# mimbres/neural-audio-fp

Hardware: NVIDIA B200
Metric: search_queries_per_s (higher is better)
Workload: dtype bf16 scan, f32 re-rank

## Files before the change

neural-audio-fp_b200/csrc/flat_search.cu:

```cuda
#include <cfloat>
#include <climits>
#include <cstdlib>
#include <cstring>
#include <algorithm>
#include <vector>

#include "index.h"
#include "ptx.cuh"

namespace nafp {

__global__ void flat_convert_rows_kernel(const float* __restrict__ x32, __nv_bfloat16* __restrict__ x16,
                                         float* __restrict__ hn, int32_t* __restrict__ maxn2, int64_t row0,
                                         int64_t n) {
    const int lane = threadIdx.x & 31;
    const int64_t warp = (static_cast<int64_t>(blockIdx.x) * blockDim.x + threadIdx.x) >> 5;
    const int64_t nwarps = (static_cast<int64_t>(gridDim.x) * blockDim.x) >> 5;
    float mx = 0.f;
    for (int64_t r = row0 + warp; r < row0 + n; r += nwarps) {
        const float4 v = reinterpret_cast<const float4*>(x32 + r * D128)[lane];
        __nv_bfloat162 a = __floats2bfloat162_rn(v.x, v.y);
        __nv_bfloat162 b = __floats2bfloat162_rn(v.z, v.w);
        uint2 packed;
        packed.x = *reinterpret_cast<uint32_t*>(&a);
// ... 1 lines not shown
        reinterpret_cast<uint2*>(x16 + r * D128)[lane] = packed;
        float ss = v.x * v.x + v.y * v.y + v.z * v.z + v.w * v.w;
#pragma unroll
        for (int o = 16; o > 0; o >>= 1) ss += __shfl_xor_sync(0xffffffffu, ss, o);
        if (lane == 0) hn[r] = 0.5f * ss;
        mx = fmaxf(mx, ss);
    }
    if (lane == 0 && mx > 0.f) atomicMax(maxn2, __float_as_int(mx));
}

__global__ void flat_fill_kernel(float* hn, int64_t from, int64_t to, float v) {
    int64_t i = from + static_cast<int64_t>(blockIdx.x) * blockDim.x + threadIdx.x;
    if (i < to) hn[i] = v;
}

__global__ void flat_prep_kernel(const float* __restrict__ q_all, const int32_t* __restrict__ src_list, int src_off,
                                 int64_t p0, int nq, int nq_pad, int grid_scan,
                                 __nv_bfloat16* __restrict__ qbf, float* __restrict__ q32,
                                 float* __restrict__ qn2, int32_t* __restrict__ Mx, int32_t* __restrict__ Tg,
                                 int32_t* __restrict__ flags, int64_t* __restrict__ gidx, int32_t* __restrict__ tile_counter) {
    const int lane = threadIdx.x & 31;
    const int row = (blockIdx.x * blockDim.x + threadIdx.x) >> 5;
    if (blockIdx.x == 0 && threadIdx.x == 0) *tile_counter = 0;
    if (row >= nq_pad) return;
    int64_t g = -1;
    if (row < nq) g = src_list ? static_cast<int64_t>(src_list[src_off + row]) : p0 + row;
    float4 v = make_float4(0.f, 0.f, 0.f, 0.f);
    if (g >= 0) v = reinterpret_cast<const float4*>(q_all + g * D128)[lane];
    __nv_bfloat162 a = __floats2bfloat162_rn(v.x, v.y);
    __nv_bfloat162 b = __floats2bfloat162_rn(v.z, v.w);
    uint2 packed;
    packed.x = *reinterpret_cast<uint32_t*>(&a);
    packed.y = *reinterpret_cast<uint32_t*>(&b);
    reinterpret_cast<uint2*>(qbf + row * D128)[lane] = packed;
    reinterpret_cast<float4*>(q32 + row * D128)[lane] = v;
    float ss = v.x * v.x + v.y * v.y + v.z * v.z + v.w * v.w;
#pragma unroll
    for (int o = 16; o > 0; o >>= 1) ss += __shfl_xor_sync(0xffffffffu, ss, o);
    if (lane == 0) {
        qn2[row] = ss;
        Tg[row] = INT_MIN;
        flags[row] = 0;
        gidx[row] = g;
    }
    for (int c = lane; c < grid_scan; c += 32) Mx[row * grid_scan + c] = INT_MIN;
}

constexpr int RING_SLOTS = 4;
constexpr int EPI_WARPS = 16;
constexpr int SCAN_THREADS = (3 + EPI_WARPS) * 32;
constexpr int TMA_WARP = EPI_WARPS + 1, MMA_WARP = EPI_WARPS + 2;
constexpr int EPI_PARTS = EPI_WARPS / 4;
constexpr int PART_COLS = SCAN_TILE / EPI_PARTS;
constexpr int SLOT_BYTES = SCAN_TILE * 128;
constexpr int BOX_BYTES = TILE_ROWS * 128;
constexpr int Q_KB_BYTES = NQ_CTA * 128;
constexpr int Q_BYTES_MAX = 2 * Q_KB_BYTES;
constexpr int H_RING = 4;
constexpr int WARM_TILES = 8;
constexpr int SCAN_SMEM = Q_BYTES_MAX + RING_SLOTS * SLOT_BYTES + H_RING * SCAN_TILE * 4 + 3 * NQ_CTA * 4 + 256 + 1024;
constexpr uint16_t PAIR_MASK = 0b11, RANK0_MASK = 0b01;
constexpr int NEG_INF_ORD = static_cast<int>(0x807FFFFFu);
static_assert(PART_COLS == 64, "epilogue reads two 32-column chunks per unit");

struct ScanBars {
    uint64_t full[RING_SLOTS];
    uint64_t empty[RING_SLOTS];
    uint64_t tfull[2];
    uint64_t tempty[2];
    uint64_t qfull;
    uint32_t tmem_base;
    int done;
    int tile_of[8];
};

__device__ __forceinline__ void smem_red_max(int* p, int v) {
    asm volatile("red.shared.max.s32 [%0], %1;" ::"r"(smem_u32(p)), "r"(v) : "memory");
}
__device__ __forceinline__ int smem_atom_inc(int* p) {
    int old;
    asm volatile("atom.shared.add.u32 %0, [%1], 1;" : "=r"(old) : "r"(smem_u32(p)) : "memory");
    return old;
}
__device__ __forceinline__ int smem_atom_add(int* p, int v) {
    int old;
    asm volatile("atom.shared.add.u32 %0, [%1], %2;" : "=r"(old) : "r"(smem_u32(p)), "r"(v) : "memory");
    return old;
}
__device__ __forceinline__ int smem_ld_volatile(const int* p) {
    int v;
    asm volatile("ld.volatile.shared.s32 %0, [%1];" : "=r"(v) : "r"(smem_u32(p)) : "memory");
    return v;
}
__device__ __forceinline__ float fmax3(float a, float b, float c) {
    float d;
    asm("max.f32 %0, %1, %2, %3;" : "=f"(d) : "f"(a), "f"(b), "f"(c));
    return d;
}
__device__ __forceinline__ void mbar_arrive_lane0(uint64_t* bar, int lane) {
    asm volatile(
        "{\n\t.reg .pred p;\n\tsetp.eq.s32 p, %1, 0;\n\t@p mbarrier.arrive.shared::cta.b64 _, [%0];\n\t}" ::"r"(smem_u32(bar)),
        "r"(lane)
        : "memory");
}
template <bool EDGE>
__device__ __forceinline__ void scan_chunk_hits(const uint32_t (&v)[32], const float* __restrict__ hc, float t_exact, int nvalid,
                                                uint32_t rbase, int* cnt_q, int* lmax_q, uint64_t* pool_q) {
    uint32_t m = 0;
    float best = -INFINITY;
#pragma unroll
    for (int j = 0; j < 32; ++j) {
        if (!EDGE || j < nvalid) {
            const float sj = __uint_as_float(v[j]) - hc[j];
            m |= (sj > t_exact) ? (1u << j) : 0u;
            best = fmaxf(best, sj);
        }
    }
    if (m) {
        smem_red_max(lmax_q, f2ord(best));
        int pos = smem_atom_add(cnt_q, __popc(m));
        while (m) {
            const int j = __ffs(m) - 1;
            m &= m - 1;
            if (pos < POOL_CAP) pool_q[pos] = rbase + j;
            ++pos;
        }
    }
}

__global__ void __launch_bounds__(SCAN_THREADS, 1)
flat_scan_kernel(const __grid_constant__ CUtensorMap tmap_q, const __grid_constant__ CUtensorMap tmap_db,
                 const float* __restrict__ hn, int32_t* __restrict__ tile_counter, int64_t n_search, int n_tiles, int nq,
                 int n_half, int kg, int32_t* __restrict__ Mx, int32_t* __restrict__ Tg, uint64_t* __restrict__ pool,
                 int32_t* __restrict__ cnt, int32_t* __restrict__ flags, int32_t* __restrict__ dbg_first, int tune) {
    extern __shared__ uint8_t smem_raw[];
    uint8_t* smem = reinterpret_cast<uint8_t*>((reinterpret_cast<uintptr_t>(smem_raw) + 1023) & ~uintptr_t(1023));
    uint8_t* q_s = smem;
    uint8_t* b_s = smem + Q_BYTES_MAX;
    float* h_s = reinterpret_cast<float*>(b_s + RING_SLOTS * SLOT_BYTES);
    int* lmax_s = reinterpret_cast<int*>(h_s + H_RING * SCAN_TILE);
    int* cnt_s = lmax_s + 2 * NQ_CTA;
    ScanBars* bars = reinterpret_cast<ScanBars*>(cnt_s + NQ_CTA);

    const int warp = threadIdx.x >> 5;
    const int lane = threadIdx.x & 31;
    const int G = gridDim.x;
    const int cta = blockIdx.x;
    const int rank = cta & 1, clu = cta >> 1, C = G >> 1;
    const int qrow0 = rank * n_half * 128;
    const int warm_cap = ((tune >> 8) & 15) ? ((tune >> 8) & 15) : WARM_TILES;
    const int warm = (tune & 2) ? 1 : max(1, min(warm_cap, n_tiles / C));

    for (int i = threadIdx.x; i < NQ_CTA; i += blockDim.x) {
        lmax_s[i] = INT_MIN;
        lmax_s[NQ_CTA + i] = INT_MIN;
        cnt_s[i] = 0;
    }
    if (threadIdx.x == 0) {
        tma_prefetch_desc(&tmap_q);
        tma_prefetch_desc(&tmap_db);
        for (int s = 0; s < RING_SLOTS; ++s) {
            mbar_init(&bars->full[s], 1);
            mbar_init(&bars->empty[s], 2);
        }
        for (int a = 0; a < 2; ++a) {
            mbar_init(&bars->tfull[a], 1);
            mbar_init(&bars->tempty[a], EPI_WARPS);
        }
        mbar_init(&bars->qfull, 1);
        bars->done = 0;
        mbar_fence_init();
    }
    if (warp == MMA_WARP) {
        tmem_alloc(&bars->tmem_base, 512);
        tmem_relinquish();
    }
    tc_fence_before();
    cluster_sync();
    tc_fence_after();
    const uint32_t tmem_base = __shfl_sync(0xffffffffu, bars->tmem_base, 0);

    if (warp == TMA_WARP) {
        if (lane == 0) {
            const int q_rows = n_half * 128;
            mbar_arrive_expect_tx(&bars->qfull, 2u * q_rows * 128u);
            for (int kb = 0; kb < 2; ++kb)
                for (int r0 = 0; r0 < q_rows; r0 += 32)
                    tma_load_2d(q_s + kb * Q_KB_BYTES + r0 * 128, &tmap_q, &bars->qfull, kb * 64, qrow0 + r0);
        }
        if (lane == 0 && rank == 0) {
            const uint32_t peer_full0 = map_shared_rank(&bars->full[0], 1);
            const uint32_t peer_tile_of0 = map_shared_rank(&bars->tile_of[0], 1);
            int tile = clu;
            int revisit = -1;
            int nxt = warm * C + atomicAdd(tile_counter, 1);
            int i = 0;
            for (;; ++i) {
                const int kc0 = 2 * i;
                const uint32_t ph = (kc0 / RING_SLOTS) & 1;
                const int s0 = kc0 % RING_SLOTS;
                mbar_wait_parked(&bars->empty[s0], ph ^ 1);
                bars->tile_of[i & 7] = tile;
                mbar_arrive_expect_tx_remote(peer_full0 + 8 * s0, (tile < 0 ? 0 : SLOT_BYTES + SCAN_TILE * 4) + 4);
                st_async_remote(peer_tile_of0 + 4 * (i & 7), tile, peer_full0 + 8 * s0);
                if (tile < 0) {
                    mbar_arrive(&bars->full[s0]);
                    break;
                }
#pragma unroll
                for (int kb = 0; kb < 2; ++kb) {
                    const int s = s0 + kb;
                    if (kb == 1) {
                        mbar_wait_parked(&bars->empty[s], ph ^ 1);
                        mbar_arrive_expect_tx_remote(peer_full0 + 8 * s, SLOT_BYTES);
                    }
                    mbar_arrive_expect_tx(&bars->full[s], SLOT_BYTES + (kb == 0 ? SCAN_TILE * 4 : 0));
                    if (kb == 0)
                        bulk_load_1d_multicast(h_s + (i % H_RING) * SCAN_TILE, hn + static_cast<int64_t>(tile) * SCAN_TILE,
                                               SCAN_TILE * 4, &bars->full[s], PAIR_MASK);
                    uint8_t* dst = b_s + s * SLOT_BYTES;
                    tma_load_2d_multicast(dst, &tmap_db, &bars->full[s], kb * 64, tile * SCAN_TILE, PAIR_MASK);
                    tma_load_2d_multicast(dst + BOX_BYTES, &tmap_db, &bars->full[s], kb * 64, tile * SCAN_TILE + TILE_ROWS,
                                          PAIR_MASK);
                }
                if (i + 1 < warm) {
                    tile = clu + (i + 1) * C;
                } else if (revisit < 0 && nxt < n_tiles) {
                    tile = nxt;
                    nxt = warm * C + atomicAdd(tile_counter, 1);
                } else {
                    ++revisit;
                    tile = revisit < warm ? clu + revisit * C : -1;
                }
            }
            for (int kc = 2 * i + 1; kc < 2 * i + RING_SLOTS; ++kc)
                mbar_wait_parked(&bars->empty[kc % RING_SLOTS], ((kc / RING_SLOTS) & 1) ^ 1);
        }
        __syncwarp();
    } else if (warp == MMA_WARP) {
        const bool leader = elect_one();
        const uint32_t idesc = umma_idesc_f16(1u, 128u, static_cast<uint32_t>(SCAN_TILE));
        const uint64_t adesc0 = umma_desc_sw128(smem_u32(q_s));
        const uint64_t bdesc0 = umma_desc_sw128(smem_u32(b_s));
        mbar_wait_parked(&bars->qfull, 0);
        uint32_t uc = 0;
        bool more = true;
        for (int i = 0; more; ++i) {
            const int s0 = (2 * i) % RING_SLOTS, s1 = s0 + 1;
            const uint32_t ph = ((2 * i) / RING_SLOTS) & 1;
            for (int hq = 0; hq < n_half; ++hq, ++uc) {
                const int acc = uc & 1;
                const uint32_t aph = (uc >> 1) & 1;
                const bool last = hq == n_half - 1;
                mbar_wait_parked(&bars->tempty[acc], aph ^ 1);
                if (hq == 0) {
                    mbar_wait_parked_cluster(&bars->full[s0], ph);
                    if (smem_ld_volatile(&bars->tile_of[i & 7]) < 0) {
                        if (leader) tc_commit(&bars->tfull[acc]);
                        __syncwarp();
                        more = false;
                        break;
                    }
                }
                tc_fence_after();
                const uint32_t d_tmem = tmem_base + acc * SCAN_TILE;
                const uint64_t a_kb0 = adesc0 + static_cast<uint64_t>((hq * (128 * 128)) >> 4);
                const uint64_t a_kb1 = a_kb0 + static_cast<uint64_t>(Q_KB_BYTES >> 4);
                const uint64_t b_kb0 = bdesc0 + static_cast<uint64_t>((s0 * SLOT_BYTES) >> 4);
                const uint64_t b_kb1 = b_kb0 + static_cast<uint64_t>(SLOT_BYTES >> 4);
                if (leader) {
#pragma unroll
                    for (int j = 0; j < 4; ++j) tc_mma_f16(d_tmem, a_kb0 + 2 * j, b_kb0 + 2 * j, idesc, j != 0 ? 1u : 0u);
                    if (last) tc_commit_multicast(&bars->empty[s0], RANK0_MASK);
                }
                if (hq == 0) {
                    mbar_wait_parked_cluster(&bars->full[s1], ph);
                    tc_fence_after();
                }
                if (leader) {
#pragma unroll
                    for (int j = 0; j < 4; ++j) tc_mma_f16(d_tmem, a_kb1 + 2 * j, b_kb1 + 2 * j, idesc, 1u);
                    if (last) tc_commit_multicast(&bars->empty[s1], RANK0_MASK);
                    tc_commit(&bars->tfull[acc]);
                }
                __syncwarp();
            }
        }
        __syncwarp();
    } else if (warp < EPI_WARPS) {
        const int qd = warp & 3;
        const int e = warp;
        const int part = e >> 2;
        constexpr int QPW = NQ_CTA / EPI_WARPS;
        static_assert(2 * QPW == 32, "one lane per (query, column half) when maxima are published");
        const int q_rows = n_half * 128;
        int* lmax_part = lmax_s + (part >> 1) * NQ_CTA;
        const float NEG_INF = -INFINITY;
        int pub = INT_MIN;
        int thr_ord[2] = {NEG_INF_ORD, NEG_INF_ORD};
        float t_exact[2], t_pre[2];
        bool active[2];
#pragma unroll
        for (int hq = 0; hq < 2; ++hq) {
            active[hq] = hq < n_half && qrow0 + (hq * 128 + qd * 32 + lane) < nq;
            t_exact[hq] = active[hq] ? NEG_INF : INFINITY;
            t_pre[hq] = t_exact[hq];
        }
        uint64_t* my_pool = pool + static_cast<int64_t>(cta) * NQ_CTA * POOL_CAP;
        const uint32_t ns32 = static_cast<uint32_t>(n_search);
        auto load_thresholds = [&](int (&tg)[2]) {
#pragma unroll
            for (int hq = 0; hq < 2; ++hq) tg[hq] = active[hq] ? ld_relaxed(&Tg[qrow0 + hq * 128 + qd * 32 + lane]) : INT_MIN;
        };
        auto apply_thresholds = [&](const int (&tg)[2], int i) -> bool {
            bool valid = true;
#pragma unroll
            for (int hq = 0; hq < 2; ++hq) {
                if (active[hq]) {
                    if (tg[hq] > thr_ord[hq]) {
                        if (dbg_first && part == 0 && thr_ord[hq] == NEG_INF_ORD)
                            dbg_first[cta * NQ_MAX + qrow0 + hq * 128 + qd * 32 + lane] = i;
                        thr_ord[hq] = tg[hq];
                        const float t = ord2f(tg[hq]);
                        t_exact[hq] = t;
                        t_pre[hq] = t - fabsf(t) * (1.f / 1048576.f) - 1e-37f;
                    }
                    valid = valid && (thr_ord[hq] > NEG_INF_ORD);
                }
            }
            return __all_sync(0xffffffffu, valid);
        };
        auto publish_maxima = [&]() {
            const int ql = e * QPW + (lane % QPW), half = lane / QPW;
            if (ql < q_rows && qrow0 + ql < nq) {
                const int m = smem_ld_volatile(&lmax_s[half * NQ_CTA + ql]);
                if (m > pub) {
                    st_relaxed(&Mx[(qrow0 + ql) * G + 2 * clu + half], m);
                    pub = m;
                }
            }
        };
        const bool probe = dbg_first != nullptr && threadIdx.x == 0 && nq <= NQ_MAX - 8;
        unsigned long long t_start = 0;
        if (probe) asm volatile("mov.u64 %0, %%globaltimer;" : "=l"(t_start));
        auto stamp = [&](int slot) {
            if (probe) {
                unsigned long long t;
                asm volatile("mov.u64 %0, %%globaltimer;" : "=l"(t));
                dbg_first[cta * NQ_MAX + NQ_MAX - 8 + slot] = static_cast<int>(t - t_start);
            }
        };
        const uint32_t tlane = tmem_base + (static_cast<uint32_t>(qd * 32) << 16) + part * PART_COLS;
        uint32_t uc = 0;

        for (int w = 0; w < warm; ++w) {
            const uint32_t row0 = static_cast<uint32_t>(clu + w * C) * SCAN_TILE + part * PART_COLS;
            const float* h_part = h_s + (w % H_RING) * SCAN_TILE + part * PART_COLS;
            bool edge = (static_cast<uint32_t>(clu + w * C) + 1u) * SCAN_TILE > ns32 || (tune & 4);
            float hx = 0.f;
            for (int hq = 0; hq < n_half; ++hq, ++uc) {
                const int acc = uc & 1;
                mbar_wait_parked(&bars->tfull[acc], (uc >> 1) & 1);
                if (hq == 0 && !edge) {
                    const float a = h_part[lane], b = h_part[32 + lane];
                    const float hmax_w = __uint_as_float(__reduce_max_sync(0xffffffffu, __float_as_uint(fmaxf(a, b))));
                    const float hmin_w = __uint_as_float(__reduce_min_sync(0xffffffffu, __float_as_uint(fminf(a, b))));
                    hx = hmax_w * (1.f + 1.f / 1048576.f);
                    edge = !(hmax_w - hmin_w <= hmax_w * (1.f / 262144.f));
                }
                tc_fence_after();
                float munit = NEG_INF;
#pragma unroll 1
                for (int c = 0; c < PART_COLS / 32; ++c) {
                    uint32_t v[32];
                    tmem_ld_32x32(tlane + acc * SCAN_TILE + c * 32, v);
                    tc_wait_ld();
                    if (!edge) {
                        float gm[4];
#pragma unroll
                        for (int g = 0; g < 4; ++g) {
                            float m = fmax3(__uint_as_float(v[8 * g]), __uint_as_float(v[8 * g + 1]), __uint_as_float(v[8 * g + 2]));
                            m = fmax3(m, __uint_as_float(v[8 * g + 3]), __uint_as_float(v[8 * g + 4]));
                            m = fmax3(m, __uint_as_float(v[8 * g + 5]), __uint_as_float(v[8 * g + 6]));
                            gm[g] = fmaxf(m, __uint_as_float(v[8 * g + 7]));
                        }
                        munit = fmaxf(munit, fmaxf(fmax3(gm[0], gm[1], gm[2]), gm[3]) - hx);
                    } else {
                        const float* hc = h_part + c * 32;
                        const int nvalid = static_cast<int>(min(ns32 - min(ns32, row0 + c * 32), 32u));
#pragma unroll
                        for (int j = 0; j < 32; ++j)
                            if (j < nvalid) munit = fmaxf(munit, __uint_as_float(v[j]) - hc[j]);
                    }
                }
                if (hq == 0 ? active[0] : active[1]) smem_red_max(&lmax_part[hq * 128 + qd * 32 + lane], f2ord(munit));
                tc_fence_before();
                __syncwarp();
                mbar_arrive_lane0(&bars->tempty[acc], lane);
            }
            publish_maxima();
            if (w == 0) stamp(0);
        }
        {
            int tg[2];
            bool ok = false;
            for (int spin = 0; spin < 4096 && !ok; ++spin) {
                publish_maxima();
                load_thresholds(tg);
                ok = apply_thresholds(tg, 1);
                if (!ok) __nanosleep(100);
            }
            stamp(1);
        }
        for (int i = warm;; ++i) {
            int tg[2] = {INT_MIN, INT_MIN};
            const bool rf = i > warm && (((tune & 8) && i < warm + 32) || (i & 3) == 0);
            if (rf) load_thresholds(tg);
            const float* h_part = h_s + (i % H_RING) * SCAN_TILE + part * PART_COLS;
            uint32_t row0 = 0;
            float hm = 0.f;
            bool end = false, edge = false;
            for (int hq = 0; hq < n_half; ++hq, ++uc) {
                const int acc = uc & 1;
                mbar_wait_parked(&bars->tfull[acc], (uc >> 1) & 1);
                if (hq == 0) {
                    const int tile = smem_ld_volatile(&bars->tile_of[i & 7]);
                    if (tile < 0) {
                        end = true;
                        break;
                    }
                    row0 = static_cast<uint32_t>(tile) * SCAN_TILE + part * PART_COLS;
                    const float hmin_w =
                        __uint_as_float(__reduce_min_sync(0xffffffffu, __float_as_uint(fminf(h_part[lane], h_part[32 + lane]))));
                    hm = hmin_w * (1.f - 1.f / 1048576.f);
                    edge = (static_cast<uint32_t>(tile) + 1u) * SCAN_TILE > ns32 || (tune & 4);
                }
                const float tp = (hq == 0 ? t_pre[0] : t_pre[1]) + hm;
                tc_fence_after();
                const uint32_t taddr = tlane + acc * SCAN_TILE;
#pragma unroll 1
                for (int c = 0; c < PART_COLS / 32; ++c) {
                    uint32_t v[32];
                    tmem_ld_32x32(taddr + c * 32, v);
                    tc_wait_ld();
                    float gm[4];
#pragma unroll
                    for (int g = 0; g < 4; ++g) {
                        float m = fmax3(__uint_as_float(v[8 * g]), __uint_as_float(v[8 * g + 1]), __uint_as_float(v[8 * g + 2]));
                        m = fmax3(m, __uint_as_float(v[8 * g + 3]), __uint_as_float(v[8 * g + 4]));
                        m = fmax3(m, __uint_as_float(v[8 * g + 5]), __uint_as_float(v[8 * g + 6]));
                        gm[g] = fmaxf(m, __uint_as_float(v[8 * g + 7]));
                    }
                    const float ma = fmaxf(fmax3(gm[0], gm[1], gm[2]), gm[3]);
                    const bool fired = ma > tp;
                    if (__any_sync(0xffffffffu, fired)) {
                        const int q = hq * 128 + qd * 32 + lane;
                        const float te = hq == 0 ? t_exact[0] : t_exact[1];
                        const uint32_t rbase = row0 + c * 32;
                        if (!edge)
                            scan_chunk_hits<false>(v, h_part + c * 32, te, 32, rbase, &cnt_s[q], &lmax_part[q], my_pool + q * POOL_CAP);
                        else
                            scan_chunk_hits<true>(v, h_part + c * 32, te, static_cast<int>(min(ns32 - min(ns32, rbase), 32u)), rbase,
                                                  &cnt_s[q], &lmax_part[q], my_pool + q * POOL_CAP);
                        __syncwarp();
                    }
                }
                tc_fence_before();
                __syncwarp();
                mbar_arrive_lane0(&bars->tempty[acc], lane);
            }
            if (end) break;
            if (rf) apply_thresholds(tg, i);
            if (i < warm + 32 || (i & 3) == 0) publish_maxima();
            if (i == warm) stamp(2);
            if (i == 16) stamp(5);
            if (i == 32) stamp(6);
            if (i == 96) stamp(7);
        }
        stamp(3);
        publish_maxima();
        stamp(4);
        __syncwarp();
        asm volatile("bar.sync 1, %0;" ::"n"(EPI_WARPS * 32) : "memory");
        {
            const int ql = e * QPW + lane;
            if (lane < QPW && ql < q_rows && qrow0 + ql < nq) {
                const int c = cnt_s[ql];
                cnt[cta * NQ_CTA + ql] = min(c, POOL_CAP);
                if (c > POOL_CAP) flags[qrow0 + ql] = 1;
            }
        }
        if (lane == 0) smem_atom_inc(&bars->done);
    } else {
        uint32_t round = 0;
        while (smem_ld_volatile(&bars->done) < EPI_WARPS) {
            for (int q = cta; q < nq; q += G) {
                uint32_t u[5];
#pragma unroll
                for (int t = 0; t < 5; ++t) {
                    const int g = lane + 32 * t;
                    const int m = g < G ? ld_relaxed(&Mx[q * G + g]) : INT_MIN;
                    u[t] = static_cast<uint32_t>(m) ^ 0x80000000u;
                }
                uint32_t res = 0;
                for (int bit = 31; bit >= 0; --bit) {
                    const uint32_t cand = res | (1u << bit);
                    int c = 0;
#pragma unroll
                    for (int t = 0; t < 5; ++t) c += (u[t] >= cand) ? 1 : 0;
                    c = __reduce_add_sync(0xffffffffu, c);
                    if (c >= kg) res = cand;
                }
                const int T = static_cast<int>(res ^ 0x80000000u);
                if (lane == 0 && T > NEG_INF_ORD && T > ld_relaxed(&Tg[q])) st_relaxed(&Tg[q], T);
            }
            ++round;
            if ((tune & 1) || round < 6) {
                __nanosleep((tune & 1) ? (round < 48 ? 100 : (round < 96 ? 1000 : 4000)) : 100);
            } else {
                for (int nap = 0; nap < 8 && smem_ld_volatile(&bars->done) < EPI_WARPS; ++nap) __nanosleep(500);
            }
        }
    }

    tc_fence_before();
    cluster_sync();
    if (warp == MMA_WARP) tmem_dealloc(tmem_base, 512);
}

__device__ __forceinline__ uint64_t score_key(float s, uint32_t row) {
    return (static_cast<uint64_t>(static_cast<uint32_t>(f2ord(s)) ^ 0x80000000u) << 32) | (0xFFFFFFFFu - row);
}
__device__ __forceinline__ float key_score(uint64_t key) {
    return ord2f(static_cast<int>(static_cast<uint32_t>(key >> 32) ^ 0x80000000u));
}
__device__ __forceinline__ uint32_t key_row(uint64_t key) { return 0xFFFFFFFFu - static_cast<uint32_t>(key); }

__device__ void bitonic_sort_desc(uint64_t* keys, int n) {
    for (int k = 2; k <= n; k <<= 1) {
        for (int j = k >> 1; j > 0; j >>= 1) {
            for (int i = threadIdx.x; i < n; i += blockDim.x) {
                const int ixj = i ^ j;
                if (ixj > i) {
                    const uint64_t a = keys[i], b = keys[ixj];
                    const bool desc = (i & k) == 0;
                    if (desc ? (a < b) : (a > b)) {
                        keys[i] = b;
                        keys[ixj] = a;
                    }
                }
            }
            __syncthreads();
        }
    }
}

struct SelBatch {
    int np[SEL_SLOTS];
    int h[SEL_SLOTS];
    int grid_alloc;
};

__global__ void __launch_bounds__(256)
flat_select_kernel(SelBatch batch, int k, int grid_scan, int64_t n_rows, const float* __restrict__ q32,
                   const float* __restrict__ qn2, const float* __restrict__ x32, const float* __restrict__ hn,
                   const int32_t* __restrict__ maxn2, const int32_t* __restrict__ Tg,
                   const uint64_t* __restrict__ pool, const int32_t* __restrict__ cnt, int32_t* __restrict__ flags,
                   const int64_t* __restrict__ gidx, int32_t* __restrict__ fail_list, int32_t* __restrict__ fail_count,
                   int64_t label_offset, float* __restrict__ D, int64_t* __restrict__ I,
                   unsigned long long* __restrict__ stats) {
    __shared__ uint64_t keys[SELECT_CAP];
    __shared__ int total_s;
    const int q = blockIdx.x;
    const int slot = blockIdx.y;
    if (q >= batch.np[slot]) return;
    q32 += static_cast<int64_t>(slot) * NQ_MAX * D128;
    qn2 += slot * NQ_MAX;
    Tg += slot * NQ_MAX;
    pool += static_cast<int64_t>(slot) * batch.grid_alloc * NQ_CTA * POOL_CAP;
    cnt += static_cast<int64_t>(slot) * batch.grid_alloc * NQ_CTA;
// ... 723 lines not shown
```

neural-audio-fp_b200/csrc/ptx.cuh:

```cuda
#pragma once
#include <cstdint>
#include <cuda_runtime.h>

namespace nafp {

__device__ __forceinline__ uint32_t smem_u32(const void* p) {
    return static_cast<uint32_t>(__cvta_generic_to_shared(p));
}

__device__ __forceinline__ bool elect_one() {
    uint32_t pred = 0;
    asm volatile(
        "{\n\t.reg .pred P;\n\t"
        "elect.sync _|P, 0xffffffff;\n\t"
        "selp.u32 %0, 1, 0, P;\n\t}\n"
        : "=r"(pred));
    return pred != 0;
}

__device__ __forceinline__ void mbar_init(uint64_t* bar, uint32_t count) {
    asm volatile("mbarrier.init.shared::cta.b64 [%0], %1;" ::"r"(smem_u32(bar)), "r"(count) : "memory");
}
__device__ __forceinline__ void mbar_fence_init() {
    asm volatile("fence.mbarrier_init.release.cluster;" ::: "memory");
// ... 36 lines not shown
        if (++spins > (1u << 24)) __trap();
    }
}
__device__ __forceinline__ void mbar_wait_parked_cluster(uint64_t* bar, uint32_t parity) {
    uint32_t spins = 0;
    for (;;) {
        uint32_t ok;
        asm volatile(
            "{\n\t.reg .pred P;\n\t"
            "mbarrier.try_wait.parity.acquire.cluster.shared::cta.b64 P, [%1], %2, %3;\n\t"
            "selp.u32 %0, 1, 0, P;\n\t}\n"
            : "=r"(ok)
            : "r"(smem_u32(bar)), "r"(parity), "r"(2000u)
            : "memory");
        if (ok) return;
        if (++spins > (1u << 24)) __trap();
    }
}

__device__ __forceinline__ void cluster_sync() {
    asm volatile("barrier.cluster.arrive.release.aligned;\n\tbarrier.cluster.wait.acquire.aligned;" ::: "memory");
}
__device__ __forceinline__ uint32_t map_shared_rank(const void* p, uint32_t rank) {
    uint32_t r;
    asm volatile("mapa.shared::cluster.u32 %0, %1, %2;" : "=r"(r) : "r"(smem_u32(p)), "r"(rank));
    return r;
}
__device__ __forceinline__ void mbar_arrive_expect_tx_remote(uint32_t bar_cluster, uint32_t bytes) {
    asm volatile("mbarrier.arrive.expect_tx.relaxed.cluster.shared::cluster.b64 _, [%0], %1;" ::"r"(bar_cluster), "r"(bytes)
                 : "memory");
}
__device__ __forceinline__ void st_async_remote(uint32_t dst_cluster, int32_t v, uint32_t bar_cluster) {
    asm volatile("st.async.shared::cluster.mbarrier::complete_tx::bytes.b32 [%0], %1, [%2];" ::"r"(dst_cluster), "r"(v),
                 "r"(bar_cluster)
                 : "memory");
}

__device__ __forceinline__ void tma_prefetch_desc(const void* tmap) {
    asm volatile("prefetch.tensormap [%0];" ::"l"(reinterpret_cast<uint64_t>(tmap)) : "memory");
}
__device__ __forceinline__ void tma_load_2d(void* smem_dst, const void* tmap, uint64_t* bar, int32_t c0, int32_t c1) {
    asm volatile(
        "cp.async.bulk.tensor.2d.shared::cluster.global.mbarrier::complete_tx::bytes [%0], [%1, {%3, %4}], [%2];"
        ::"r"(smem_u32(smem_dst)), "l"(reinterpret_cast<uint64_t>(tmap)), "r"(smem_u32(bar)), "r"(c0), "r"(c1)
        : "memory");
}
__device__ __forceinline__ void tma_load_2d_multicast(void* smem_dst, const void* tmap, uint64_t* bar, int32_t c0, int32_t c1,
                                                      uint16_t cta_mask) {
    asm volatile(
        "cp.async.bulk.tensor.2d.shared::cluster.global.mbarrier::complete_tx::bytes.multicast::cluster [%0], [%1, {%3, %4}], [%2], %5;"
        ::"r"(smem_u32(smem_dst)), "l"(reinterpret_cast<uint64_t>(tmap)), "r"(smem_u32(bar)), "r"(c0), "r"(c1), "h"(cta_mask)
        : "memory");
}
__device__ __forceinline__ void tma_load_3d(void* smem_dst, const void* tmap, uint64_t* bar, int32_t c0, int32_t c1, int32_t c2) {
    asm volatile(
        "cp.async.bulk.tensor.3d.shared::cluster.global.mbarrier::complete_tx::bytes [%0], [%1, {%3, %4, %5}], [%2];"
        ::"r"(smem_u32(smem_dst)), "l"(reinterpret_cast<uint64_t>(tmap)), "r"(smem_u32(bar)), "r"(c0), "r"(c1), "r"(c2)
        : "memory");
}
__device__ __forceinline__ void tma_load_4d(void* smem_dst, const void* tmap, uint64_t* bar, int32_t c0, int32_t c1, int32_t c2, int32_t c3) {
    asm volatile(
        "cp.async.bulk.tensor.4d.shared::cluster.global.mbarrier::complete_tx::bytes [%0], [%1, {%3, %4, %5, %6}], [%2];"
        ::"r"(smem_u32(smem_dst)), "l"(reinterpret_cast<uint64_t>(tmap)), "r"(smem_u32(bar)), "r"(c0), "r"(c1), "r"(c2), "r"(c3)
        : "memory");
}
__device__ __forceinline__ void tma_load_5d(void* smem_dst, const void* tmap, uint64_t* bar, int32_t c0, int32_t c1, int32_t c2, int32_t c3, int32_t c4) {
    asm volatile(
        "cp.async.bulk.tensor.5d.shared::cluster.global.mbarrier::complete_tx::bytes [%0], [%1, {%3, %4, %5, %6, %7}], [%2];"
        ::"r"(smem_u32(smem_dst)), "l"(reinterpret_cast<uint64_t>(tmap)), "r"(smem_u32(bar)), "r"(c0), "r"(c1), "r"(c2), "r"(c3), "r"(c4)
        : "memory");
}
__device__ __forceinline__ void tma_store_2d(const void* tmap, const void* smem_src, int32_t c0, int32_t c1) {
    asm volatile("cp.async.bulk.tensor.2d.global.shared::cta.bulk_group [%0, {%2, %3}], [%1];"
                 ::"l"(reinterpret_cast<uint64_t>(tmap)), "r"(smem_u32(smem_src)), "r"(c0), "r"(c1) : "memory");
}
__device__ __forceinline__ void tma_store_commit() { asm volatile("cp.async.bulk.commit_group;" ::: "memory"); }
__device__ __forceinline__ void tma_store_wait_read() { asm volatile("cp.async.bulk.wait_group.read 0;" ::: "memory"); }
__device__ __forceinline__ void tma_store_wait_all() { asm volatile("cp.async.bulk.wait_group 0;" ::: "memory"); }
__device__ __forceinline__ uint64_t pk2(float a, float b) {
    uint64_t r;
    asm("mov.b64 %0, {%1, %2};" : "=l"(r) : "f"(a), "f"(b));
    return r;
}
__device__ __forceinline__ void upk2(uint64_t v, float& a, float& b) { asm("mov.b64 {%0, %1}, %2;" : "=f"(a), "=f"(b) : "l"(v)); }
__device__ __forceinline__ uint64_t fma2(uint64_t a, uint64_t b, uint64_t c) {
    uint64_t r;
    asm("fma.rn.f32x2 %0, %1, %2, %3;" : "=l"(r) : "l"(a), "l"(b), "l"(c));
    return r;
}
__device__ __forceinline__ uint64_t mul2(uint64_t a, uint64_t b) {
    uint64_t r;
    asm("mul.rn.f32x2 %0, %1, %2;" : "=l"(r) : "l"(a), "l"(b));
    return r;
}
__device__ __forceinline__ uint64_t add2(uint64_t a, uint64_t b) {
    uint64_t r;
    asm("add.rn.f32x2 %0, %1, %2;" : "=l"(r) : "l"(a), "l"(b));
    return r;
}

__device__ __forceinline__ void bulk_load_1d(void* smem_dst, const void* gsrc, uint32_t bytes, uint64_t* bar) {
    asm volatile("cp.async.bulk.shared::cluster.global.mbarrier::complete_tx::bytes [%0], [%1], %2, [%3];" ::"r"(smem_u32(smem_dst)),
                 "l"(reinterpret_cast<uint64_t>(gsrc)), "r"(bytes), "r"(smem_u32(bar))
                 : "memory");
}
__device__ __forceinline__ void bulk_load_1d_multicast(void* smem_dst, const void* gsrc, uint32_t bytes, uint64_t* bar,
                                                       uint16_t cta_mask) {
    asm volatile("cp.async.bulk.shared::cluster.global.mbarrier::complete_tx::bytes.multicast::cluster [%0], [%1], %2, [%3], %4;"
                 ::"r"(smem_u32(smem_dst)), "l"(reinterpret_cast<uint64_t>(gsrc)), "r"(bytes), "r"(smem_u32(bar)), "h"(cta_mask)
                 : "memory");
}
__device__ __forceinline__ void fence_proxy_async_smem() {
    asm volatile("fence.proxy.async.shared::cta;" ::: "memory");
}

__device__ __forceinline__ void tmem_alloc(uint32_t* smem_result, uint32_t ncols) {
    asm volatile("tcgen05.alloc.cta_group::1.sync.aligned.shared::cta.b32 [%0], %1;" ::"r"(smem_u32(smem_result)), "r"(ncols) : "memory");
}
__device__ __forceinline__ void tmem_relinquish() {
    asm volatile("tcgen05.relinquish_alloc_permit.cta_group::1.sync.aligned;" ::: "memory");
}
__device__ __forceinline__ void tmem_dealloc(uint32_t taddr, uint32_t ncols) {
    asm volatile("tcgen05.dealloc.cta_group::1.sync.aligned.b32 %0, %1;" ::"r"(taddr), "r"(ncols) : "memory");
}
__device__ __forceinline__ void tc_fence_before() { asm volatile("tcgen05.fence::before_thread_sync;" ::: "memory"); }
__device__ __forceinline__ void tc_fence_after() { asm volatile("tcgen05.fence::after_thread_sync;" ::: "memory"); }
__device__ __forceinline__ void tc_wait_ld() { asm volatile("tcgen05.wait::ld.sync.aligned;" ::: "memory"); }

__device__ __forceinline__ void tc_mma_f16(uint32_t tmem_d, uint64_t adesc, uint64_t bdesc, uint32_t idesc, uint32_t accumulate) {
    asm volatile(
        "{\n\t.reg .pred p;\n\t"
        "setp.ne.b32 p, %4, 0;\n\t"
        "tcgen05.mma.cta_group::1.kind::f16 [%0], %1, %2, %3, p;\n\t}\n"
        ::"r"(tmem_d), "l"(adesc), "l"(bdesc), "r"(idesc), "r"(accumulate)
        : "memory");
}
__device__ __forceinline__ void tc_commit(uint64_t* bar) {
    asm volatile("tcgen05.commit.cta_group::1.mbarrier::arrive::one.shared::cluster.b64 [%0];" ::"r"(smem_u32(bar)) : "memory");
}
__device__ __forceinline__ void tc_commit_multicast(uint64_t* bar, uint16_t cta_mask) {
    asm volatile("tcgen05.commit.cta_group::1.mbarrier::arrive::one.shared::cluster.multicast::cluster.b64 [%0], %1;"
                 ::"r"(smem_u32(bar)), "h"(cta_mask)
                 : "memory");
}

__device__ __forceinline__ void tmem_ld_32x32(uint32_t taddr, uint32_t (&v)[32]) {
    asm volatile(
        "tcgen05.ld.sync.aligned.32x32b.x32.b32 "
        "{%0, %1, %2, %3, %4, %5, %6, %7, %8, %9, %10, %11, %12, %13, %14, %15, "
        "%16, %17, %18, %19, %20, %21, %22, %23, %24, %25, %26, %27, %28, %29, %30, %31}, [%32];"
        : "=r"(v[0]), "=r"(v[1]), "=r"(v[2]), "=r"(v[3]), "=r"(v[4]), "=r"(v[5]), "=r"(v[6]), "=r"(v[7]),
          "=r"(v[8]), "=r"(v[9]), "=r"(v[10]), "=r"(v[11]), "=r"(v[12]), "=r"(v[13]), "=r"(v[14]), "=r"(v[15]),
          "=r"(v[16]), "=r"(v[17]), "=r"(v[18]), "=r"(v[19]), "=r"(v[20]), "=r"(v[21]), "=r"(v[22]), "=r"(v[23]),
          "=r"(v[24]), "=r"(v[25]), "=r"(v[26]), "=r"(v[27]), "=r"(v[28]), "=r"(v[29]), "=r"(v[30]), "=r"(v[31])
        : "r"(taddr)
        : "memory");
}
__device__ __forceinline__ void tmem_ld_32x64(uint32_t taddr, uint32_t (&v)[64]) {
    asm volatile(
        "tcgen05.ld.sync.aligned.32x32b.x64.b32 "
        "{%0, %1, %2, %3, %4, %5, %6, %7, %8, %9, %10, %11, %12, %13, %14, %15, %16, %17, %18, %19, %20, %21, %22, %23, %24, %25, %26, %27, %28, %29, %30, %31, %32, %33, %34, %35, %36, %37, %38, %39, %40, %41, %42, %43, %44, %45, %46, %47, %48, %49, %50, %51, %52, %53, %54, %55, %56, %57, %58, %59, %60, %61, %62, %63}, [%64];"
        : "=r"(v[0]), "=r"(v[1]), "=r"(v[2]), "=r"(v[3]), "=r"(v[4]), "=r"(v[5]), "=r"(v[6]), "=r"(v[7]), "=r"(v[8]), "=r"(v[9]), "=r"(v[10]), "=r"(v[11]), "=r"(v[12]), "=r"(v[13]), "=r"(v[14]), "=r"(v[15]), "=r"(v[16]), "=r"(v[17]), "=r"(v[18]), "=r"(v[19]), "=r"(v[20]), "=r"(v[21]), "=r"(v[22]), "=r"(v[23]), "=r"(v[24]), "=r"(v[25]), "=r"(v[26]), "=r"(v[27]), "=r"(v[28]), "=r"(v[29]), "=r"(v[30]), "=r"(v[31]), "=r"(v[32]), "=r"(v[33]), "=r"(v[34]), "=r"(v[35]), "=r"(v[36]), "=r"(v[37]), "=r"(v[38]), "=r"(v[39]), "=r"(v[40]), "=r"(v[41]), "=r"(v[42]), "=r"(v[43]), "=r"(v[44]), "=r"(v[45]), "=r"(v[46]), "=r"(v[47]), "=r"(v[48]), "=r"(v[49]), "=r"(v[50]), "=r"(v[51]), "=r"(v[52]), "=r"(v[53]), "=r"(v[54]), "=r"(v[55]), "=r"(v[56]), "=r"(v[57]), "=r"(v[58]), "=r"(v[59]), "=r"(v[60]), "=r"(v[61]), "=r"(v[62]), "=r"(v[63])
        : "r"(taddr)
        : "memory");
}
__device__ __forceinline__ uint32_t tmem_ld_32x1(uint32_t taddr) {
    uint32_t v;
    asm volatile("tcgen05.ld.sync.aligned.32x32b.x1.b32 {%0}, [%1];" : "=r"(v) : "r"(taddr) : "memory");
    return v;
}
__device__ __forceinline__ void tmem_ld_32x16(uint32_t taddr, uint32_t (&v)[16]) {
    asm volatile(
        "tcgen05.ld.sync.aligned.32x32b.x16.b32 "
        "{%0, %1, %2, %3, %4, %5, %6, %7, %8, %9, %10, %11, %12, %13, %14, %15}, [%16];"
        : "=r"(v[0]), "=r"(v[1]), "=r"(v[2]), "=r"(v[3]), "=r"(v[4]), "=r"(v[5]), "=r"(v[6]), "=r"(v[7]),
          "=r"(v[8]), "=r"(v[9]), "=r"(v[10]), "=r"(v[11]), "=r"(v[12]), "=r"(v[13]), "=r"(v[14]), "=r"(v[15])
        : "r"(taddr)
        : "memory");
}

__device__ __forceinline__ void tmem_st_32x16(uint32_t taddr, const uint32_t (&v)[16]) {
    asm volatile(
        "tcgen05.st.sync.aligned.32x32b.x16.b32 [%0], "
        "{%1, %2, %3, %4, %5, %6, %7, %8, %9, %10, %11, %12, %13, %14, %15, %16};"
        ::"r"(taddr), "r"(v[0]), "r"(v[1]), "r"(v[2]), "r"(v[3]), "r"(v[4]), "r"(v[5]), "r"(v[6]), "r"(v[7]),
          "r"(v[8]), "r"(v[9]), "r"(v[10]), "r"(v[11]), "r"(v[12]), "r"(v[13]), "r"(v[14]), "r"(v[15])
        : "memory");
}
__device__ __forceinline__ void tc_wait_st() { asm volatile("tcgen05.wait::st.sync.aligned;" ::: "memory"); }

__device__ __forceinline__ uint64_t umma_desc_sw128(uint32_t smem_addr) {
    uint64_t d = 0;
    d |= static_cast<uint64_t>((smem_addr & 0x3FFFFu) >> 4);
    d |= static_cast<uint64_t>(1) << 16;
// ... 35 lines not shown
```

Measured before the change: 43540.

## Switch scan GEMM to paired-CTA tcgen05 MMA with split DB tiles

Converts the two-CTA cluster scan from independent cta_group::1 MMAs, each with a full multicast DB tile, to a single cta_group::2 MMA issued by rank 0. Each CTA now holds half the DB tile and the queries are split across the pair. Norm loads move onto a separate per-slot ifull barrier ring with a deeper H_RING. The epilogue reads 64 TMEM columns in one load and releases the accumulator before doing the threshold work. The aim is to halve per-CTA shared-memory traffic and MMA issue, and to overlap accumulator reuse with the epilogue. This adds cross-CTA barrier coupling and more register pressure from the 64-element load.

Result: slower. 41570 (median of 6 runs) (-4.5%).

```diff
diff --git a/neural-audio-fp_b200/csrc/flat_search.cu b/neural-audio-fp_b200/csrc/flat_search.cu
--- a/neural-audio-fp_b200/csrc/flat_search.cu
+++ b/neural-audio-fp_b200/csrc/flat_search.cu
@@ -77,14 +77,13 @@
 constexpr int TMA_WARP = EPI_WARPS + 1, MMA_WARP = EPI_WARPS + 2;
 constexpr int EPI_PARTS = EPI_WARPS / 4;
 constexpr int PART_COLS = SCAN_TILE / EPI_PARTS;
-constexpr int SLOT_BYTES = SCAN_TILE * 128;
-constexpr int BOX_BYTES = TILE_ROWS * 128;
+constexpr int SLOT_BYTES = TILE_ROWS * 128;
 constexpr int Q_KB_BYTES = NQ_CTA * 128;
 constexpr int Q_BYTES_MAX = 2 * Q_KB_BYTES;
-constexpr int H_RING = 4;
+constexpr int H_RING = 8;
 constexpr int WARM_TILES = 8;
 constexpr int SCAN_SMEM = Q_BYTES_MAX + RING_SLOTS * SLOT_BYTES + H_RING * SCAN_TILE * 4 + 3 * NQ_CTA * 4 + 256 + 1024;
-constexpr uint16_t PAIR_MASK = 0b11, RANK0_MASK = 0b01;
+constexpr uint16_t PAIR_MASK = 0b11, RANK0_MASK = 0b01, PEER_MASK = 0b10;
 constexpr int NEG_INF_ORD = static_cast<int>(0x807FFFFFu);
 static_assert(PART_COLS == 64, "epilogue reads two 32-column chunks per unit");
 
@@ -93,6 +92,7 @@
     uint64_t empty[RING_SLOTS];
     uint64_t tfull[2];
     uint64_t tempty[2];
+    uint64_t ifull[H_RING];
     uint64_t qfull;
     uint32_t tmem_base;
     int done;
@@ -122,9 +122,9 @@
     asm("max.f32 %0, %1, %2, %3;" : "=f"(d) : "f"(a), "f"(b), "f"(c));
     return d;
 }
-__device__ __forceinline__ void mbar_arrive_lane0(uint64_t* bar, int lane) {
+__device__ __forceinline__ void mbar_arrive_lane0(uint32_t bar_cluster, int lane) {
     asm volatile(
-        "{\n\t.reg .pred p;\n\tsetp.eq.s32 p, %1, 0;\n\t@p mbarrier.arrive.shared::cta.b64 _, [%0];\n\t}" ::"r"(smem_u32(bar)),
+        "{\n\t.reg .pred p;\n\tsetp.eq.s32 p, %1, 0;\n\t@p mbarrier.arrive.shared::cluster.b64 _, [%0];\n\t}" ::"r"(bar_cluster),
         "r"(lane)
         : "memory");
 }
@@ -186,19 +186,20 @@
         tma_prefetch_desc(&tmap_db);
         for (int s = 0; s < RING_SLOTS; ++s) {
             mbar_init(&bars->full[s], 1);
-            mbar_init(&bars->empty[s], 2);
+            mbar_init(&bars->empty[s], 1);
         }
         for (int a = 0; a < 2; ++a) {
             mbar_init(&bars->tfull[a], 1);
-            mbar_init(&bars->tempty[a], EPI_WARPS);
-        }
+            mbar_init(&bars->tempty[a], 2 * EPI_WARPS);
+        }
+        for (int h = 0; h < H_RING; ++h) mbar_init(&bars->ifull[h], 1);
         mbar_init(&bars->qfull, 1);
         bars->done = 0;
         mbar_fence_init();
     }
     if (warp == MMA_WARP) {
-        tmem_alloc(&bars->tmem_base, 512);
-        tmem_relinquish();
+        tmem_alloc_pair(&bars->tmem_base, 512);
+        tmem_relinquish_pair();
     }
     tc_fence_before();
     cluster_sync();
@@ -206,15 +207,16 @@
     const uint32_t tmem_base = __shfl_sync(0xffffffffu, bars->tmem_base, 0);
 
     if (warp == TMA_WARP) {
-        if (lane == 0) {
+        if (lane == 0 && rank == 0) {
             const int q_rows = n_half * 128;
-            mbar_arrive_expect_tx(&bars->qfull, 2u * q_rows * 128u);
+            mbar_arrive_expect_tx(&bars->qfull, 2u * 2u * q_rows * 128u);
             for (int kb = 0; kb < 2; ++kb)
-                for (int r0 = 0; r0 < q_rows; r0 += 32)
-                    tma_load_2d(q_s + kb * Q_KB_BYTES + r0 * 128, &tmap_q, &bars->qfull, kb * 64, qrow0 + r0);
-        }
-        if (lane == 0 && rank == 0) {
-            const uint32_t peer_full0 = map_shared_rank(&bars->full[0], 1);
+                for (int r0 = 0; r0 < q_rows; r0 += 32) {
+                    tma_load_2d(q_s + kb * Q_KB_BYTES + r0 * 128, &tmap_q, &bars->qfull, kb * 64, r0);
+                    tma_load_2d_multicast_pair(q_s + kb * Q_KB_BYTES + r0 * 128, &tmap_q, &bars->qfull, kb * 64, q_rows + r0,
+                                               PEER_MASK);
+                }
+            const uint32_t peer_ifull0 = map_shared_rank(&bars->ifull[0], 1);
             const uint32_t peer_tile_of0 = map_shared_rank(&bars->tile_of[0], 1);
             int tile = clu;
             int revisit = -1;
@@ -224,29 +226,27 @@
                 const int kc0 = 2 * i;
                 const uint32_t ph = (kc0 / RING_SLOTS) & 1;
                 const int s0 = kc0 % RING_SLOTS;
+                const int hb = i % H_RING;
                 mbar_wait_parked(&bars->empty[s0], ph ^ 1);
                 bars->tile_of[i & 7] = tile;
-                mbar_arrive_expect_tx_remote(peer_full0 + 8 * s0, (tile < 0 ? 0 : SLOT_BYTES + SCAN_TILE * 4) + 4);
-                st_async_remote(peer_tile_of0 + 4 * (i & 7), tile, peer_full0 + 8 * s0);
+                mbar_arrive_expect_tx_remote(peer_ifull0 + 8 * hb, (tile < 0 ? 0 : SCAN_TILE * 4) + 4);
+                st_async_remote(peer_tile_of0 + 4 * (i & 7), tile, peer_ifull0 + 8 * hb);
                 if (tile < 0) {
+                    mbar_arrive(&bars->ifull[hb]);
                     mbar_arrive(&bars->full[s0]);
                     break;
                 }
+                mbar_arrive_expect_tx(&bars->ifull[hb], SCAN_TILE * 4);
+                bulk_load_1d_multicast(h_s + hb * SCAN_TILE, hn + static_cast<int64_t>(tile) * SCAN_TILE, SCAN_TILE * 4,
+                                       &bars->ifull[hb], PAIR_MASK);
 #pragma unroll
                 for (int kb = 0; kb < 2; ++kb) {
                     const int s = s0 + kb;
-                    if (kb == 1) {
-                        mbar_wait_parked(&bars->empty[s], ph ^ 1);
-                        mbar_arrive_expect_tx_remote(peer_full0 + 8 * s, SLOT_BYTES);
-                    }
-                    mbar_arrive_expect_tx(&bars->full[s], SLOT_BYTES + (kb == 0 ? SCAN_TILE * 4 : 0));
-                    if (kb == 0)
-                        bulk_load_1d_multicast(h_s + (i % H_RING) * SCAN_TILE, hn + static_cast<int64_t>(tile) * SCAN_TILE,
-                                               SCAN_TILE * 4, &bars->full[s], PAIR_MASK);
+                    if (kb == 1) mbar_wait_parked(&bars->empty[s], ph ^ 1);
+                    mbar_arrive_expect_tx(&bars->full[s], 2 * SLOT_BYTES);
                     uint8_t* dst = b_s + s * SLOT_BYTES;
-                    tma_load_2d_multicast(dst, &tmap_db, &bars->full[s], kb * 64, tile * SCAN_TILE, PAIR_MASK);
-                    tma_load_2d_multicast(dst + BOX_BYTES, &tmap_db, &bars->full[s], kb * 64, tile * SCAN_TILE + TILE_ROWS,
-                                          PAIR_MASK);
+                    tma_load_2d(dst, &tmap_db, &bars->full[s], kb * 64, tile * SCAN_TILE);
+                    tma_load_2d_multicast_pair(dst, &tmap_db, &bars->full[s], kb * 64, tile * SCAN_TILE + TILE_ROWS, PEER_MASK);
                 }
                 if (i + 1 < warm) {
                     tile = clu + (i + 1) * C;
@@ -263,52 +263,52 @@
         }
         __syncwarp();
     } else if (warp == MMA_WARP) {
-        const bool leader = elect_one();
-        const uint32_t idesc = umma_idesc_f16(1u, 128u, static_cast<uint32_t>(SCAN_TILE));
-        const uint64_t adesc0 = umma_desc_sw128(smem_u32(q_s));
-        const uint64_t bdesc0 = umma_desc_sw128(smem_u32(b_s));
-        mbar_wait_parked(&bars->qfull, 0);
-        uint32_t uc = 0;
-        bool more = true;
-        for (int i = 0; more; ++i) {
-            const int s0 = (2 * i) % RING_SLOTS, s1 = s0 + 1;
-            const uint32_t ph = ((2 * i) / RING_SLOTS) & 1;
-            for (int hq = 0; hq < n_half; ++hq, ++uc) {
-                const int acc = uc & 1;
-                const uint32_t aph = (uc >> 1) & 1;
-                const bool last = hq == n_half - 1;
-                mbar_wait_parked(&bars->tempty[acc], aph ^ 1);
-                if (hq == 0) {
-                    mbar_wait_parked_cluster(&bars->full[s0], ph);
-                    if (smem_ld_volatile(&bars->tile_of[i & 7]) < 0) {
-                        if (leader) tc_commit(&bars->tfull[acc]);
-                        __syncwarp();
-                        more = false;
-                        break;
+        if (rank == 0) {
+            const bool leader = elect_one();
+            const uint32_t idesc = umma_idesc_f16(1u, 256u, static_cast<uint32_t>(SCAN_TILE));
+            const uint64_t adesc0 = umma_desc_sw128(smem_u32(q_s));
+            const uint64_t bdesc0 = umma_desc_sw128(smem_u32(b_s));
+            mbar_wait_parked(&bars->qfull, 0);
+            uint32_t uc = 0;
+            bool more = true;
+            for (int i = 0; more; ++i) {
+                const int s0 = (2 * i) % RING_SLOTS, s1 = s0 + 1;
+                const uint32_t ph = ((2 * i) / RING_SLOTS) & 1;
+                for (int hq = 0; hq < n_half; ++hq, ++uc) {
+                    const int acc = uc & 1;
+                    const uint32_t aph = (uc >> 1) & 1;
+                    const bool last = hq == n_half - 1;
+                    mbar_wait_parked(&bars->tempty[acc], aph ^ 1);
+                    if (hq == 0) {
+                        mbar_wait_parked_cluster(&bars->full[s0], ph);
+                        if (smem_ld_volatile(&bars->tile_of[i & 7]) < 0) {
+                            more = false;
+                            break;
+                        }
                     }
+                    tc_fence_after();
+                    const uint32_t d_tmem = tmem_base + acc * SCAN_TILE;
+                    const uint64_t a_kb0 = adesc0 + static_cast<uint64_t>((hq * (128 * 128)) >> 4);
+                    const uint64_t a_kb1 = a_kb0 + static_cast<uint64_t>(Q_KB_BYTES >> 4);
+                    const uint64_t b_kb0 = bdesc0 + static_cast<uint64_t>((s0 * SLOT_BYTES) >> 4);
+                    const uint64_t b_kb1 = b_kb0 + static_cast<uint64_t>(SLOT_BYTES >> 4);
+                    if (leader) {
+#pragma unroll
+                        for (int j = 0; j < 4; ++j) tc_mma_f16_pair(d_tmem, a_kb0 + 2 * j, b_kb0 + 2 * j, idesc, j != 0 ? 1u : 0u);
+                        if (last) tc_commit_pair_multicast(&bars->empty[s0], RANK0_MASK);
+                    }
+                    if (hq == 0) {
+                        mbar_wait_parked_cluster(&bars->full[s1], ph);
+                        tc_fence_after();
+                    }
+                    if (leader) {
+#pragma unroll
+                        for (int j = 0; j < 4; ++j) tc_mma_f16_pair(d_tmem, a_kb1 + 2 * j, b_kb1 + 2 * j, idesc, 1u);
+                        if (last) tc_commit_pair_multicast(&bars->empty[s1], RANK0_MASK);
+                        tc_commit_pair_multicast(&bars->tfull[acc], PAIR_MASK);
+                    }
+                    __syncwarp();
                 }
-                tc_fence_after();
-                const uint32_t d_tmem = tmem_base + acc * SCAN_TILE;
-                const uint64_t a_kb0 = adesc0 + static_cast<uint64_t>((hq * (128 * 128)) >> 4);
-                const uint64_t a_kb1 = a_kb0 + static_cast<uint64_t>(Q_KB_BYTES >> 4);
-                const uint64_t b_kb0 = bdesc0 + static_cast<uint64_t>((s0 * SLOT_BYTES) >> 4);
-                const uint64_t b_kb1 = b_kb0 + static_cast<uint64_t>(SLOT_BYTES >> 4);
-                if (leader) {
-#pragma unroll
-                    for (int j = 0; j < 4; ++j) tc_mma_f16(d_tmem, a_kb0 + 2 * j, b_kb0 + 2 * j, idesc, j != 0 ? 1u : 0u);
-                    if (last) tc_commit_multicast(&bars->empty[s0], RANK0_MASK);
-                }
-                if (hq == 0) {
-                    mbar_wait_parked_cluster(&bars->full[s1], ph);
-                    tc_fence_after();
-                }
-                if (leader) {
-#pragma unroll
-                    for (int j = 0; j < 4; ++j) tc_mma_f16(d_tmem, a_kb1 + 2 * j, b_kb1 + 2 * j, idesc, 1u);
-                    if (last) tc_commit_multicast(&bars->empty[s1], RANK0_MASK);
-                    tc_commit(&bars->tfull[acc]);
-                }
-                __syncwarp();
             }
         }
         __syncwarp();
@@ -376,11 +376,13 @@
             }
         };
         const uint32_t tlane = tmem_base + (static_cast<uint32_t>(qd * 32) << 16) + part * PART_COLS;
+        const uint32_t tempty0 = map_shared_rank(&bars->tempty[0], 0);
         uint32_t uc = 0;
 
         for (int w = 0; w < warm; ++w) {
             const uint32_t row0 = static_cast<uint32_t>(clu + w * C) * SCAN_TILE + part * PART_COLS;
             const float* h_part = h_s + (w % H_RING) * SCAN_TILE + part * PART_COLS;
+            mbar_wait_parked_cluster(&bars->ifull[w % H_RING], (w / H_RING) & 1);
             bool edge = (static_cast<uint32_t>(clu + w * C) + 1u) * SCAN_TILE > ns32 || (tune & 4);
             float hx = 0.f;
             for (int hq = 0; hq < n_half; ++hq, ++uc) {
@@ -421,7 +423,7 @@
                 if (hq == 0 ? active[0] : active[1]) smem_red_max(&lmax_part[hq * 128 + qd * 32 + lane], f2ord(munit));
                 tc_fence_before();
                 __syncwarp();
-                mbar_arrive_lane0(&bars->tempty[acc], lane);
+                mbar_arrive_lane0(tempty0 + 8 * acc, lane);
             }
             publish_maxima();
             if (w == 0) stamp(0);
@@ -442,39 +444,35 @@
             const bool rf = i > warm && (((tune & 8) && i < warm + 32) || (i & 3) == 0);
             if (rf) load_thresholds(tg);
             const float* h_part = h_s + (i % H_RING) * SCAN_TILE + part * PART_COLS;
-            uint32_t row0 = 0;
-            float hm = 0.f;
-            bool end = false, edge = false;
+            mbar_wait_parked_cluster(&bars->ifull[i % H_RING], (i / H_RING) & 1);
+            const int tile = smem_ld_volatile(&bars->tile_of[i & 7]);
+            if (tile < 0) break;
+            const uint32_t row0 = static_cast<uint32_t>(tile) * SCAN_TILE + part * PART_COLS;
+            const float hmin_w =
+                __uint_as_float(__reduce_min_sync(0xffffffffu, __float_as_uint(fminf(h_part[lane], h_part[32 + lane]))));
+            const float hm = hmin_w * (1.f - 1.f / 1048576.f);
+            const bool edge = (static_cast<uint32_t>(tile) + 1u) * SCAN_TILE > ns32 || (tune & 4);
             for (int hq = 0; hq < n_half; ++hq, ++uc) {
                 const int acc = uc & 1;
                 mbar_wait_parked(&bars->tfull[acc], (uc >> 1) & 1);
-                if (hq == 0) {
-                    const int tile = smem_ld_volatile(&bars->tile_of[i & 7]);
-                    if (tile < 0) {
-                        end = true;
-                        break;
-                    }
-                    row0 = static_cast<uint32_t>(tile) * SCAN_TILE + part * PART_COLS;
-                    const float hmin_w =
-                        __uint_as_float(__reduce_min_sync(0xffffffffu, __float_as_uint(fminf(h_part[lane], h_part[32 + lane]))));
-                    hm = hmin_w * (1.f - 1.f / 1048576.f);
-                    edge = (static_cast<uint32_t>(tile) + 1u) * SCAN_TILE > ns32 || (tune & 4);
-                }
                 const float tp = (hq == 0 ? t_pre[0] : t_pre[1]) + hm;
                 tc_fence_after();
-                const uint32_t taddr = tlane + acc * SCAN_TILE;
-#pragma unroll 1
+                uint32_t v[64];
+                tmem_ld_32x64(tlane + acc * SCAN_TILE, v);
+                tc_wait_ld();
+                tc_fence_before();
+                __syncwarp();
+                mbar_arrive_lane0(tempty0 + 8 * acc, lane);
+#pragma unroll
                 for (int c = 0; c < PART_COLS / 32; ++c) {
-                    uint32_t v[32];
-                    tmem_ld_32x32(taddr + c * 32, v);
-                    tc_wait_ld();
+                    const uint32_t (&vc)[32] = *reinterpret_cast<const uint32_t(*)[32]>(&v[32 * c]);
                     float gm[4];
 #pragma unroll
                     for (int g = 0; g < 4; ++g) {
-                        float m = fmax3(__uint_as_float(v[8 * g]), __uint_as_float(v[8 * g + 1]), __uint_as_float(v[8 * g + 2]));
-                        m = fmax3(m, __uint_as_float(v[8 * g + 3]), __uint_as_float(v[8 * g + 4]));
-                        m = fmax3(m, __uint_as_float(v[8 * g + 5]), __uint_as_float(v[8 * g + 6]));
-                        gm[g] = fmaxf(m, __uint_as_float(v[8 * g + 7]));
+                        float m = fmax3(__uint_as_float(vc[8 * g]), __uint_as_float(vc[8 * g + 1]), __uint_as_float(vc[8 * g + 2]));
+                        m = fmax3(m, __uint_as_float(vc[8 * g + 3]), __uint_as_float(vc[8 * g + 4]));
+                        m = fmax3(m, __uint_as_float(vc[8 * g + 5]), __uint_as_float(vc[8 * g + 6]));
+                        gm[g] = fmaxf(m, __uint_as_float(vc[8 * g + 7]));
                     }
                     const float ma = fmaxf(fmax3(gm[0], gm[1], gm[2]), gm[3]);
                     const bool fired = ma > tp;
@@ -483,18 +481,14 @@
                         const float te = hq == 0 ? t_exact[0] : t_exact[1];
                         const uint32_t rbase = row0 + c * 32;
                         if (!edge)
-                            scan_chunk_hits<false>(v, h_part + c * 32, te, 32, rbase, &cnt_s[q], &lmax_part[q], my_pool + q * POOL_CAP);
+                            scan_chunk_hits<false>(vc, h_part + c * 32, te, 32, rbase, &cnt_s[q], &lmax_part[q], my_pool + q * POOL_CAP);
                         else
-                            scan_chunk_hits<true>(v, h_part + c * 32, te, static_cast<int>(min(ns32 - min(ns32, rbase), 32u)), rbase,
+                            scan_chunk_hits<true>(vc, h_part + c * 32, te, static_cast<int>(min(ns32 - min(ns32, rbase), 32u)), rbase,
                                                   &cnt_s[q], &lmax_part[q], my_pool + q * POOL_CAP);
                         __syncwarp();
                     }
                 }
-                tc_fence_before();
-                __syncwarp();
-                mbar_arrive_lane0(&bars->tempty[acc], lane);
-            }
-            if (end) break;
+            }
             if (rf) apply_thresholds(tg, i);
             if (i < warm + 32 || (i & 3) == 0) publish_maxima();
             if (i == warm) stamp(2);
@@ -550,7 +544,7 @@
 
     tc_fence_before();
     cluster_sync();
-    if (warp == MMA_WARP) tmem_dealloc(tmem_base, 512);
+    if (warp == MMA_WARP) tmem_dealloc_pair(tmem_base, 512);
 }
 
 __device__ __forceinline__ uint64_t score_key(float s, uint32_t row) {
diff --git a/neural-audio-fp_b200/csrc/ptx.cuh b/neural-audio-fp_b200/csrc/ptx.cuh
--- a/neural-audio-fp_b200/csrc/ptx.cuh
+++ b/neural-audio-fp_b200/csrc/ptx.cuh
@@ -112,6 +112,13 @@
         ::"r"(smem_u32(smem_dst)), "l"(reinterpret_cast<uint64_t>(tmap)), "r"(smem_u32(bar)), "r"(c0), "r"(c1), "h"(cta_mask)
         : "memory");
 }
+__device__ __forceinline__ void tma_load_2d_multicast_pair(void* smem_dst, const void* tmap, uint64_t* bar, int32_t c0, int32_t c1,
+                                                           uint16_t cta_mask) {
+    asm volatile(
+        "cp.async.bulk.tensor.2d.cta_group::2.shared::cluster.global.mbarrier::complete_tx::bytes.multicast::cluster [%0], [%1, {%3, %4}], [%2], %5;"
+        ::"r"(smem_u32(smem_dst)), "l"(reinterpret_cast<uint64_t>(tmap)), "r"(smem_u32(bar)), "r"(c0), "r"(c1), "h"(cta_mask)
+        : "memory");
+}
 __device__ __forceinline__ void tma_load_3d(void* smem_dst, const void* tmap, uint64_t* bar, int32_t c0, int32_t c1, int32_t c2) {
     asm volatile(
         "cp.async.bulk.tensor.3d.shared::cluster.global.mbarrier::complete_tx::bytes [%0], [%1, {%3, %4, %5}], [%2];"
@@ -183,6 +190,15 @@
 __device__ __forceinline__ void tmem_dealloc(uint32_t taddr, uint32_t ncols) {
     asm volatile("tcgen05.dealloc.cta_group::1.sync.aligned.b32 %0, %1;" ::"r"(taddr), "r"(ncols) : "memory");
 }
+__device__ __forceinline__ void tmem_alloc_pair(uint32_t* smem_result, uint32_t ncols) {
+    asm volatile("tcgen05.alloc.cta_group::2.sync.aligned.shared::cta.b32 [%0], %1;" ::"r"(smem_u32(smem_result)), "r"(ncols) : "memory");
+}
+__device__ __forceinline__ void tmem_relinquish_pair() {
+    asm volatile("tcgen05.relinquish_alloc_permit.cta_group::2.sync.aligned;" ::: "memory");
+}
+__device__ __forceinline__ void tmem_dealloc_pair(uint32_t taddr, uint32_t ncols) {
+    asm volatile("tcgen05.dealloc.cta_group::2.sync.aligned.b32 %0, %1;" ::"r"(taddr), "r"(ncols) : "memory");
+}
 __device__ __forceinline__ void tc_fence_before() { asm volatile("tcgen05.fence::before_thread_sync;" ::: "memory"); }
 __device__ __forceinline__ void tc_fence_after() { asm volatile("tcgen05.fence::after_thread_sync;" ::: "memory"); }
 __device__ __forceinline__ void tc_wait_ld() { asm volatile("tcgen05.wait::ld.sync.aligned;" ::: "memory"); }
@@ -195,11 +211,25 @@
         ::"r"(tmem_d), "l"(adesc), "l"(bdesc), "r"(idesc), "r"(accumulate)
         : "memory");
 }
+__device__ __forceinline__ void tc_mma_f16_pair(uint32_t tmem_d, uint64_t adesc, uint64_t bdesc, uint32_t idesc, uint32_t accumulate) {
+    asm volatile(
+        "{\n\t.reg .pred p;\n\t"
+        "setp.ne.b32 p, %4, 0;\n\t"
+        "tcgen05.mma.cta_group::2.kind::f16 [%0], %1, %2, %3, p;\n\t}\n"
+        ::"r"(tmem_d), "l"(adesc), "l"(bdesc), "r"(idesc), "r"(accumulate)
+        : "memory");
+}
 __device__ __forceinline__ void tc_commit(uint64_t* bar) {
     asm volatile("tcgen05.commit.cta_group::1.mbarrier::arrive::one.shared::cluster.b64 [%0];" ::"r"(smem_u32(bar)) : "memory");
 }
 __device__ __forceinline__ void tc_commit_multicast(uint64_t* bar, uint16_t cta_mask) {
     asm volatile("tcgen05.commit.cta_group::1.mbarrier::arrive::one.shared::cluster.multicast::cluster.b64 [%0], %1;"
+                 ::"r"(smem_u32(bar)), "h"(cta_mask)
+                 : "memory");
+}
+
+__device__ __forceinline__ void tc_commit_pair_multicast(uint64_t* bar, uint16_t cta_mask) {
+    asm volatile("tcgen05.commit.cta_group::2.mbarrier::arrive::one.shared::cluster.multicast::cluster.b64 [%0], %1;"
                  ::"r"(smem_u32(bar)), "h"(cta_mask)
                  : "memory");
 }
```
